# shadimsaleh/motion_detection

Measured on AMD Instinct MI355X. Metric: Mpixels/s (flow+warp+diff) at 1080p & 4K; % HBM roofline, 1/2/4/8 GPU, higher is better.
Workload: dtype u8

## Files before the change

motion_detection_amd/csrc/mdx_api.cpp:

```cpp
#include "mdx_ctx.h"

#include <cstdlib>
#include <map>
#include <mutex>

using namespace mdx;

static thread_local std::string g_create_err;

extern "C" void mdx_default_params(mdx_params* p)
{
    p->win = 40;
    p->max_level = 5;
    p->max_iters = 10;
    p->eps = 0.03;
    p->min_eig = 0.001f;
    p->thresh = 190;
    p->pixel_step = 10;
    p->min_vector_size = 1.0;
    p->fit_mode = MDX_FIT_FIRST4;
    p->subspace_precision = MDX_SUBSPACE_F64;
    p->call_pipelining = 0;
    p->ransac_iters = 128;
    p->ransac_thresh = 3.0;
    p->ransac_seed = 20141105u;
}

extern "C" int mdx_grid_count(int w, int h, int ps)
{
    if (w <= 0 || h <= 0 || ps <= 0) return 0;
    return ((w + ps - 1) / ps) * ((h + ps - 1) / ps);
}

static const char* check_params(const mdx_params* p)
{
    if (p->win != kWin) return "only win == 40 (the reference constant) is supported";
    if (p->max_level < 0 || p->max_level >= kMaxLevels) return "max_level out of range [0, 7]";
    if (p->pixel_step <= 0) return "pixel_step must be > 0 (reference leaves it unset: UB)";
    if (p->fit_mode != MDX_FIT_FIRST4 && p->fit_mode != MDX_FIT_EXTERNAL && p->fit_mode != MDX_FIT_RANSAC) return "bad fit_mode";
    if (p->ransac_iters < 1 || p->ransac_iters > kRansacMaxIters) return "ransac_iters must be in [1, 1024]";
    if (!(p->ransac_thresh >= 0.0) || !(p->ransac_thresh < 1e6)) return "ransac_thresh must be in [0, 1e6)";
    if (p->subspace_precision != MDX_SUBSPACE_F64 && p->subspace_precision != MDX_SUBSPACE_F32) return "bad subspace_precision";
    if (p->call_pipelining != 0 && p->call_pipelining != 1) return "call_pipelining must be 0 or 1";
    return nullptr;
}

static std::mutex g_host_mu;
static std::map<uintptr_t, size_t> g_host_blocks;
bool mdx::host_block_holds(const void* p, size_t bytes)
{
    const uintptr_t a = reinterpret_cast<uintptr_t>(p);
    std::lock_guard<std::mutex> lk(g_host_mu);
    auto it = g_host_blocks.upper_bound(a);
    if (it == g_host_blocks.begin()) return false;
    --it;
    return a >= it->first && bytes <= it->second && a - it->first <= it->second - bytes;
}

extern "C" const char* mdx_create_error(void) { return g_create_err.c_str(); }
extern "C" int mdx_abi_version(void) { return MDX_ABI_VERSION; }
extern "C" size_t mdx_params_size(void) { return sizeof(mdx_params); }

static LkTuning read_tuning()
{
    LkTuning t;
    auto num = [](const char* name, int dflt) {
        const char* e = std::getenv(name);
        return e ? std::atoi(e) : dflt;
    };
    t.lk_impl = num("MDX_LK_IMPL", 2) == 1 ? 1 : 2;
    t.lk_g = num("MDX_LK_G", 0);
    t.lk_sub = num("MDX_LK_SUB", 0);
    t.lk_astrip = std::max(0, std::min(num("MDX_LK_ASTRIP", 0), 64));
    t.lk_debug = num("MDX_LK_DEBUG", 0) != 0;
    t.traj_chain = num("MDX_TRAJ_CHAIN", 1) != 0;
    const int ppw = num("MDX_TRAJ_PPW", 4);
    t.traj_ppw = ppw == 1 ? 1 : ppw == 2 ? 2 : 4;
    t.lk_aux = num("MDX_LK_AUX", 1) != 0;
    t.lk_flow = num("MDX_LK_FLOW", 1) != 0;
    t.ol_reg = num("MDX_OL_REG", 1) != 0;
    t.lk_cap = std::min(std::max(num("MDX_LK_CAP", 75), 10), 100);
    t.lk_fma = num("MDX_LK_FMA", 1) != 0;
    t.spin_max = num("MDX_LK_SPIN_MAX", kLkSpinDefault);
    return t;
}

static bool new_stream(mdx_ctx* c, hipStream_t* s)
{
    if (hipStreamCreateWithFlags(s, hipStreamNonBlocking) != hipSuccess) {
        *s = nullptr;
        return false;
    }
    c->streams.push_back(*s);
    return true;
}

static bool new_events(mdx_ctx* c, hipEvent_t* e, int n, unsigned flags = hipEventDisableTiming)
{
    for (int i = 0; i < n; i++) {
        if (hipEventCreateWithFlags(&e[i], flags) != hipSuccess) return false;
        c->events.push_back(e[i]);
    }
    return true;
}

extern "C" mdx_ctx* mdx_create(int device, int max_w, int max_h, int max_batch, const mdx_params* p)
{
    g_create_err.clear();
    mdx_params prm;
    if (p) prm = *p;
    else mdx_default_params(&prm);
    if (const char* why = check_params(&prm)) { g_create_err = why; return nullptr; }
    if (max_w <= 0 || max_h <= 0 || max_batch <= 0) { g_create_err = "max_w/max_h/max_batch must be > 0"; return nullptr; }
    int ndev = 0;
    if (hipGetDeviceCount(&ndev) != hipSuccess || ndev == 0) { g_create_err = "no HIP device visible"; return nullptr; }
    if (device < 0 || device >= ndev) { g_create_err = "device index out of range"; return nullptr; }
    if (hipSetDevice(device) != hipSuccess) { g_create_err = "hipSetDevice failed"; return nullptr; }
    mdx_ctx* c = new mdx_ctx();
    c->device = device;
    c->prm = prm;
    c->max_w = max_w;
    c->max_h = max_h;
    c->max_batch = max_batch;
    static_cast<LkTuning&>(*c) = read_tuning();
    auto fail = [&](const std::string& msg) -> mdx_ctx* {
// ... 310 lines not shown
```

motion_detection_amd/csrc/mdx_ctx.h:

```cpp
#pragma once

#include "../../include/mdx.h"
#include "mdx_internal.h"

#include <algorithm>
#include <array>
#include <cstdarg>
#include <cstdio>
#include <initializer_list>
#include <string>
#include <utility>
#include <vector>

struct DevBuf {
    void* p = nullptr;
    size_t cap = 0;
    DevBuf() = default;
    DevBuf(DevBuf&& o) noexcept : p(std::exchange(o.p, nullptr)), cap(std::exchange(o.cap, 0)) {}
    DevBuf& operator=(DevBuf&& o) noexcept
    {
        std::swap(p, o.p), std::swap(cap, o.cap);
        return *this;
    }
    ~DevBuf() { reset(); }
    void reset()
    {
        if (p) (void)hipFree(p);
        p = nullptr, cap = 0;
    }
    bool alloc(size_t bytes)
    {
        reset();
        if (hipMalloc(&p, bytes) != hipSuccess) p = nullptr;
        cap = p ? bytes : 0;
        return p != nullptr;
    }
    template <typename T> T* as() const { return static_cast<T*>(p); }
};

struct LkTuning {
    int lk_impl = 2;
    int lk_g = 0;
    int lk_sub = 0;
    int lk_astrip = 0;
    bool lk_debug = false;
    bool traj_chain = true;
    int traj_ppw = 4;
    bool lk_aux = true;
    bool lk_flow = true;
    int lk_cap = 75;
    bool lk_fma = true;
    int spin_max = mdx::kLkSpinDefault;
    bool ol_reg = true;
};

struct mdx_ctx : LkTuning {
    int device = 0;
    std::vector<hipStream_t> streams;
    std::vector<hipEvent_t> events;
    std::vector<void*> pinned;
    hipStream_t stream = nullptr;
    hipStream_t aux = nullptr;
    hipEvent_t lkev[mdx::kMaxLevels + 2] = {};
    hipStream_t iter2 = nullptr;
    hipEvent_t flowev[2] = {};
    hipEvent_t front_ev = nullptr;
    hipEvent_t pyr_free[2] = {};
    hipEvent_t lvl_done[mdx::kMaxLevels] = {};
    hipEvent_t redo_ev[mdx::kMaxLevels] = {};
    mdx::LkLaunch lk;
    int pyr_half = 0;
    hipEvent_t input_ev = nullptr;
    uint8_t* last_pyr1 = nullptr;
    uint8_t* last_pyr2 = nullptr;
    uint8_t* band_pyr1 = nullptr;
    uint8_t* band_pyr2 = nullptr;
    int band_half = 0;
    const uint8_t* band_img1 = nullptr;
    int band_built[2] = {0, 0};
    int band_stride = 0, band_fmt = 0;
    DevBuf errw;
    int* err_host = nullptr;
    int* tcnt_host = nullptr;
    long long lk_fallback[3] = {0, 0, 0};
    mdx_params prm{};
    int max_w = 0, max_h = 0, max_batch = 0;
    DevBuf pyr1, pyr2, der, fits;
    DevBuf in1, in2, np, st, vec, mask, H, Hext, num;
    DevBuf bnp, bst;
    DevBuf cls, Abuf, ctab;
    DevBuf dbg;
    DevBuf lkcnt;
    DevBuf csum;
    DevBuf tin, tcur, tnp, tst, ttraj, tnum, tflag;
    DevBuf straj, sdata, sq, scnt, scols, sres, sout, sbest;
    DevBuf clpts, clbest, clroot;
// ... 145 lines not shown
```

motion_detection_amd/csrc/mdx_dev.h:

```cpp
#pragma once

#include "mdx_internal.h"

namespace mdx {

__device__ __forceinline__ int r101(int p, int len)
{
    if ((unsigned)p < (unsigned)len) return p;
    if (len == 1) return 0;
    do {
        if (p < 0) p = -p;
        else p = 2 * len - 2 - p;
    } while ((unsigned)p >= (unsigned)len);
    return p;
}

struct __attribute__((aligned(4))) u4a4k { uint32_t x, y, z, w; };
struct __attribute__((aligned(4))) u3a4k { uint32_t x, y, z; };
struct __attribute__((aligned(4))) u2a4k { uint32_t x, y; };
template <typename T>
__device__ __forceinline__ T gload(uintptr_t a)
{
#if defined(__HIP_DEVICE_COMPILE__)
    return *reinterpret_cast<const __attribute__((address_space(1))) T*>(a);
#else
    return *reinterpret_cast<const T*>(a);
#endif
}

template <int T>
__device__ __forceinline__ int block_scan_exclusive(int v, int* wsum, int& total)
{
    const int lane = threadIdx.x & 63, w = threadIdx.x >> 6;
    int inc = v;
#pragma unroll
    for (int d = 1; d < 64; d <<= 1) {
        const int o = __shfl_up(inc, d, 64);
        if (lane >= d) inc += o;
    }
    if (lane == 63) wsum[w] = inc;
    __syncthreads();
    int off = 0, tot = 0;
#pragma unroll
    for (int i = 0; i < T / 64; i++) {
        const int s = wsum[i];
        if (i < w) off += s;
        tot += s;
    }
    __syncthreads();
    total = tot;
    return off + inc - v;
}

__device__ __forceinline__ int u8_at(const uint32_t (&w)[3], int b) { return (int)((w[b >> 2] >> (8 * (b & 3))) & 255u); }

__device__ __forceinline__ uint32_t scharr_word(const uint32_t (&ra)[3], const uint32_t (&rb)[3], const uint32_t (&rc)[3],
                                                int bc)
{
    const int bm = bc - 1, bp = bc + 1;
    const int t0m = (u8_at(ra, bm) + u8_at(rc, bm)) * 3 + u8_at(rb, bm) * 10;
    const int t0p = (u8_at(ra, bp) + u8_at(rc, bp)) * 3 + u8_at(rb, bp) * 10;
    const int t1m = u8_at(rc, bm) - u8_at(ra, bm), t1c = u8_at(rc, bc) - u8_at(ra, bc), t1p = u8_at(rc, bp) - u8_at(ra, bp);
    const int ix = t0p - t0m;
    const int iy = (t1m + t1p) * 3 + t1c * 10;
    return (uint32_t)(uint16_t)(int16_t)ix | ((uint32_t)(uint16_t)(int16_t)iy << 16);
}

__device__ __forceinline__ int gray_of(const uint8_t* s, int fmt)
{
    if (fmt == 1) return (s[0] * 1868 + s[1] * 9617 + s[2] * 4899 + 8192) >> 14;
    return (s[2] * 1868 + s[1] * 9617 + s[0] * 4899 + 8192) >> 14;
}

__device__ __forceinline__ void gray_chunk(const uint8_t* s, int px0, int w, int fmt, uint32_t (&o)[4])
{
    if (px0 >= 0 && px0 + 16 <= w && fmt == 0 && (((uintptr_t)(s + px0)) & 3) == 0) {
        const u4a4k v = *reinterpret_cast<const u4a4k*>(s + px0);
        o[0] = v.x; o[1] = v.y; o[2] = v.z; o[3] = v.w;
    } else if (px0 >= 0 && px0 + 16 <= w && fmt != 0 && (((uintptr_t)(s + 3 * px0)) & 3) == 0) {
        uint32_t b[12];
        const u4a4k* q = reinterpret_cast<const u4a4k*>(s + 3 * px0);
#pragma unroll
        for (int t = 0; t < 3; t++) { const u4a4k v = q[t]; b[4 * t] = v.x; b[4 * t + 1] = v.y; b[4 * t + 2] = v.z; b[4 * t + 3] = v.w; }
        const uint8_t* bb = reinterpret_cast<const uint8_t*>(b);
#pragma unroll
        for (int t = 0; t < 4; t++) {
            uint32_t d = 0;
#pragma unroll
            for (int i = 0; i < 4; i++) d |= (uint32_t)gray_of(bb + 3 * (4 * t + i), fmt) << (8 * i);
            o[t] = d;
        }
    } else {
        for (int t = 0; t < 4; t++) {
            uint32_t d = 0;
            for (int i = 0; i < 4; i++) {
                const int px = px0 + 4 * t + i;
                if (px < -kPad || px >= w + kPad) continue;
                const int sx = r101(px, w);
                d |= (uint32_t)(fmt == 0 ? s[sx] : gray_of(s + 3 * sx, fmt)) << (8 * i);
            }
            o[t] = d;
        }
    }
}

}
```

motion_detection_amd/csrc/mdx_internal.h:

```cpp
#pragma once

#include <hip/hip_runtime.h>
#include <math.h>
#include <stdint.h>

#include <algorithm>

#include "mdx.h"
#include "mdx_plan.h"

namespace mdx {

static_assert(sizeof(float4) == kFloat4Bytes, "lk_scratch sizes the A sums by it");
constexpr int kLkDbgStampOff = kMaxLevels * 64 + 64;
constexpr int kLkDbgWaves = 16384;

inline uint8_t* level0_core(uint8_t* slab, const Geometry& g) { return slab + g.lv[0].img_off + g.lv[0].core(); }

struct PairFit {
    double H[9];
    double Hinv[9];
    int num_vectors;
    int fit_status;
    int src_y0, src_y1;
};

struct LkClassArgs {
    Geometry g;
    ClassPlan plan;
    const int16_t* rlist;
    int level;
};

struct LkArgs {
    const uint8_t* pyr1;
    const uint8_t* pyr2;
    const uint32_t* der;
    Geometry g;
    int maxl;
    int npts, ny, pixel_step;
    int nyg;
    int max_iters;
    float min_eig;
    double eps2;
    float* next_pts;
    float* carry;
    long long carry_lstride;
    uint8_t* status;
    ClassPlan plan;
    const int16_t* cmap;
    const int16_t* rlist;
    const int16_t* ord;
    const float* prev_pts;
    int max_sub;
    int* done;
    int done_stride;
    int dep_groups;
    int* err;
    int* lflags;
    int redo;
    int spin_max;
    int flow_cap;
    float4* dbg;
    int dbg_pt;
    int fma;
    uint32_t* body_cnt;
};

constexpr int kLkSpinDefault = 1 << 19;
#ifndef MDX_LK_REDO_WAVES
#define MDX_LK_REDO_WAVES 512
#endif
constexpr int kLkRedoWaves = MDX_LK_REDO_WAVES;

hipError_t launch_gray_pad(hipStream_t s, int batch, const uint8_t* in1, const uint8_t* in2, int w, int h,
                           int stride, long long frame_stride, int fmt, uint8_t* pyr1, uint8_t* pyr2,
                           const Geometry& g, int fsel = 0);
hipError_t launch_front(hipStream_t s, int batch, const uint8_t* in1, const uint8_t* in2, int w, int h, int stride,
                        long long frame_stride, int fmt, uint8_t* pyr1, uint8_t* pyr2, const Geometry& g,
                        int fsel = 0, const RowSpan* rows = nullptr);
hipError_t launch_pyr_levels(hipStream_t s, int batch, uint8_t* pyr1, uint8_t* pyr2, const Geometry& g, int fsel = 0,
                             const RowSpan* rows = nullptr);
hipError_t launch_scharr_levels(hipStream_t s, int batch, const uint8_t* pyr1, uint32_t* der, const Geometry& g);
hipError_t launch_scharr(hipStream_t s, int batch, const uint8_t* pyr1, uint32_t* der, const Geometry& g, int level,
                         int prow0 = 0, int prow1 = -1);
hipError_t launch_lk(hipStream_t s, int batch, const LkArgs& a);

constexpr int kMaxTrajImgs = 16;
struct TrajChain {
    const uint8_t* pyr[kMaxTrajImgs];
    const uint32_t* der[kMaxTrajImgs];
    int nimg, w, h;
    float* cur;
    float* traj;
    int* tlen;
    int* flag;
    double* vectors;
    float* start_pts;
    int* num;
    double mvs;
    float* htraj;
    int* htlen;
    float* hstart;
    double* hvec;
};
hipError_t launch_lk_chain(hipStream_t s, const LkArgs& a, const TrajChain& t, int ppw);
size_t subspace_basis_bytes(int n, int d, int precision);
// ... 165 lines not shown
```

motion_detection_amd/csrc/mdx_lk.hip:

```cpp
#include "mdx_dev.h"

#include <float.h>

#include <algorithm>
#include <atomic>
#include <cstdlib>
#include <type_traits>

namespace mdx {

typedef short s2 __attribute__((ext_vector_type(2)));
typedef float f2 __attribute__((ext_vector_type(2)));
typedef unsigned int v4u __attribute__((ext_vector_type(4)));
typedef unsigned int v3u __attribute__((ext_vector_type(3)));
struct LkRunRsrc {
    unsigned long long base;
    uint32_t bytes;

    __device__ __forceinline__ LkRunRsrc(const void* p, uint32_t n)
    {
        const unsigned long long b = (unsigned long long)(uintptr_t)p;
        const uint32_t lo = __builtin_amdgcn_readfirstlane((uint32_t)b);
        const uint32_t hi = __builtin_amdgcn_readfirstlane((uint32_t)(b >> 32)) & 0xffffu;
        base = ((unsigned long long)hi << 32) | lo;
        bytes = __builtin_amdgcn_readfirstlane(n);
    }
    __device__ __forceinline__ void advance(uint32_t step)
    {
        base += step;
        bytes -= step;
        asm("" : "+s"(base), "+s"(bytes));
    }
    __device__ __forceinline__ __amdgpu_buffer_rsrc_t rsrc() const
    {
        const v4u w = {(uint32_t)base, (uint32_t)(base >> 32), bytes, 0x00020000u};
        __amdgpu_buffer_rsrc_t r;
        static_assert(sizeof(r) == sizeof(w), "descriptor words");
        __builtin_memcpy(&r, &w, sizeof(r));
        return r;
    }
};

__device__ __forceinline__ int class_of(const int16_t* cmap, int level, int axis, int res)
{
    return cmap[(level * 2 + axis) * kTabStride + res];
}
__device__ __forceinline__ int residue_of(const int16_t* rlist, int level, int axis, int cls)
{
    return rlist[(level * 2 + axis) * kTabStride + cls];
}

__device__ __forceinline__ void lk_weights(float fa, float fb, int& w00, int& w01, int& w10, int& w11)
{
    w00 = __float2int_rn((1.f - fa) * (1.f - fb) * 16384.f);
    w01 = __float2int_rn(fa * (1.f - fb) * 16384.f);
    w10 = __float2int_rn((1.f - fa) * fb * 16384.f);
    w11 = 16384 - w00 - w01 - w10;
}

template <int Q>
__device__ __forceinline__ void lk_interp(uint32_t lo0, uint32_t hi0, uint32_t lo1, uint32_t hi1, uint32_t d00,
                                          uint32_t d01, uint32_t d10, uint32_t d11, s2 W0, s2 W1, int& ival, int& ixv,
                                          int& iyv)
{
    static_assert(Q >= 0 && Q < 7, "tap byte");
    constexpr unsigned sel = 0x0c000c00u | (unsigned)Q | ((unsigned)(Q + 1) << 16);
    const s2 t0 = __builtin_bit_cast(s2, __builtin_amdgcn_perm(hi0, lo0, sel));
    const s2 t1 = __builtin_bit_cast(s2, __builtin_amdgcn_perm(hi1, lo1, sel));
    ival = __builtin_amdgcn_sdot2(t0, W0, __builtin_amdgcn_sdot2(t1, W1, 256, false), false) >> 9;
    const s2 x0 = __builtin_bit_cast(s2, __builtin_amdgcn_perm(d01, d00, 0x05040100u));
    const s2 x1 = __builtin_bit_cast(s2, __builtin_amdgcn_perm(d11, d10, 0x05040100u));
    const s2 y0 = __builtin_bit_cast(s2, __builtin_amdgcn_perm(d01, d00, 0x07060302u));
    const s2 y1 = __builtin_bit_cast(s2, __builtin_amdgcn_perm(d11, d10, 0x07060302u));
    ixv = __builtin_amdgcn_sdot2(x0, W0, __builtin_amdgcn_sdot2(x1, W1, 8192, false), false) >> 14;
    iyv = __builtin_amdgcn_sdot2(y0, W0, __builtin_amdgcn_sdot2(y1, W1, 8192, false), false) >> 14;
}

template <int J>
__device__ __forceinline__ float quad_bcast(float v)
{
    constexpr int ctrl = J | (J << 2) | (J << 4) | (J << 6);
    return __int_as_float(__builtin_amdgcn_mov_dpp(__float_as_int(v), ctrl, 0xf, 0xf, false));
}
template <int J>
__device__ __forceinline__ uint32_t quad_bcast_u(uint32_t v)
{
    constexpr int ctrl = J | (J << 2) | (J << 4) | (J << 6);
    return (uint32_t)__builtin_amdgcn_mov_dpp((int)v, ctrl, 0xf, 0xf, false);
}

__device__ __forceinline__ void wave_lds_fence()
{
    __builtin_amdgcn_fence(__ATOMIC_RELEASE, "wavefront");
    __builtin_amdgcn_wave_barrier();
    __builtin_amdgcn_fence(__ATOMIC_ACQUIRE, "wavefront");
}

constexpr int kLkIterWavesPerEU = 4;
typedef __attribute__((address_space(3))) void* lds_ptr;
typedef __attribute__((address_space(3))) uint32_t lds_u32;
typedef unsigned int v2u __attribute__((ext_vector_type(2)));
typedef __attribute__((address_space(3))) volatile const v2u lds_u2v;
typedef __attribute__((address_space(3))) volatile const v4u lds_u4v;
__device__ __forceinline__ void lk_vmcnt0()
{
    __builtin_amdgcn_sched_barrier(0);
    __builtin_amdgcn_s_waitcnt(0x0F70);
    __builtin_amdgcn_sched_barrier(0);
}
template <int N>
__device__ __forceinline__ void lk_vmcnt()
{
    static_assert(N >= 0 && N < 16, "vmcnt field");
    __builtin_amdgcn_sched_barrier(0);
    __builtin_amdgcn_s_waitcnt(0x0F70 | N);
    __builtin_amdgcn_sched_barrier(0);
}

template <int B, int E, typename F>
__device__ __forceinline__ void static_for(F&& f)
{
    if constexpr (B < E) {
        f(std::integral_constant<int, B>{});
        static_for<B + 1, E>(f);
    }
}

__device__ __forceinline__ int xcd_remap(int b, int total)
{
    const int xcd = b & 7, q = total >> 3, r = total & 7;
    return (xcd < r ? xcd * (q + 1) : r * (q + 1) + (xcd - r) * q) + (b >> 3);
}

__device__ __forceinline__ void cls_store(uint4* o, const uint32_t (&dv)[4], const int (&cv)[4])
{
    typedef unsigned v4nt __attribute__((ext_vector_type(4)));
    const uint4 a = make_uint4(dv[0], (uint32_t)cv[0], dv[1], (uint32_t)cv[1]);
    const uint4 b = make_uint4(dv[2], (uint32_t)cv[2], dv[3], (uint32_t)cv[3]);
    __builtin_nontemporal_store(__builtin_bit_cast(v4nt, a), reinterpret_cast<v4nt*>(o));
    __builtin_nontemporal_store(__builtin_bit_cast(v4nt, b), reinterpret_cast<v4nt*>(o) + 1);
}

__global__ __launch_bounds__(256) void k_lk_class(const uint8_t* __restrict__ pyr1, const uint32_t* __restrict__ der,
                                                  uint8_t* __restrict__ cls_out, LkClassArgs a)
{
    const int level = a.level;
    const ClassLevel& C = a.plan.lv[level];
    const int nclass = C.nrx * C.nry;
    const int pair = blockIdx.z / nclass, cls = blockIdx.z % nclass;
    const int j = blockIdx.x * blockDim.x + threadIdx.x;
    const int v = C.vlo + blockIdx.y;
    if (4 * j >= a.g.lv[level].w + 2 * kPad || v >= C.UH) return;
    const Level L = a.g.lv[level];
    const float scale = (float)(1. / (1 << level));
    const int rx = residue_of(a.rlist, level, 0, cls % C.nrx), ry = residue_of(a.rlist, level, 1, cls / C.nrx);
    const float ppx = (float)rx * scale - 19.5f, ppy = (float)ry * scale - 19.5f;
    const float fa = ppx - floorf(ppx), fb = ppy - floorf(ppy);
    int w00, w01, w10, w11;
    lk_weights(fa, fb, w00, w01, w10, w11);
    const uint8_t* I = pyr1 + (long long)pair * a.g.img_bytes + L.img_off + L.core();
    const uint32_t* D = der + (long long)pair * a.g.der_words + L.der_off + L.core();
    const int y = v - kPad;
    const int p = L.pitch;
    uint8_t* base = cls_out + (long long)pair * a.plan.bytes_per_pair + C.off + (long long)cls * C.class_bytes;
    uint32_t dv[4] = {0, 0, 0, 0};
    int cv[4];
    const int x0 = 4 * j - kPad;
    if (y < L.h + kPad - 1 && x0 < L.w + kPad - 1) {
        const uint8_t* ip = I + (long long)y * p + x0;
        const uint32_t* dp = D + (long long)y * p + x0;
        uint32_t ib[2][2], dw[2][5];
#pragma unroll
        for (int r = 0; r < 2; r++) {
            const u2a4k bi = *reinterpret_cast<const u2a4k*>(ip + (long long)r * p);
            ib[r][0] = bi.x; ib[r][1] = bi.y;
            const uint4 d4 = *reinterpret_cast<const uint4*>(dp + (long long)r * p);
            dw[r][0] = d4.x; dw[r][1] = d4.y; dw[r][2] = d4.z; dw[r][3] = d4.w;
            dw[r][4] = dp[(long long)r * p + 4];
        }
        const s2 W0 = {(short)w00, (short)w01}, W1 = {(short)w10, (short)w11};
        static_for<0, 4>([&](auto qc) {
            constexpr int q = decltype(qc)::value;
            if (x0 + q >= L.w + kPad - 1) { cv[q] = 256; return; }
            int ival, ixv, iyv;
            lk_interp<q>(ib[0][0], ib[0][1], ib[1][0], ib[1][1], dw[0][q], dw[0][q + 1], dw[1][q], dw[1][q + 1], W0, W1,
                         ival, ixv, iyv);
            dv[q] = ((uint32_t)ixv & 0xffffu) | ((uint32_t)iyv << 16);
            cv[q] = 256 - 512 * ival;
        });
    } else {
#pragma unroll
        for (int q = 0; q < 4; q++) cv[q] = 256;
    }
    uint4* o = reinterpret_cast<uint4*>(base) + ((long long)v * C.PW + 4 * j) / 2;
    cls_store(o, dv, cv);
}

__global__ __launch_bounds__(256) void k_lk_class_fused(const uint8_t* __restrict__ pyr1, uint8_t* __restrict__ cls_out,
                                                        LkClassArgs a)
{
    const int level = a.level;
    const ClassLevel& C = a.plan.lv[level];
    const int nclass = C.nrx * C.nry;
    const int pair = blockIdx.z;
    const int j = blockIdx.x * blockDim.x + threadIdx.x;
    const int v = C.vlo + blockIdx.y;
    if (4 * j >= a.g.lv[level].w + 2 * kPad || v >= C.UH) return;
    const Level L = a.g.lv[level];
    const float scale = (float)(1. / (1 << level));
    const uint8_t* I = pyr1 + (long long)pair * a.g.img_bytes + L.img_off + L.core();
    const int y = v - kPad;
    const int p = L.pitch;
    const int x0 = 4 * j - kPad;
    const bool inside = y < L.h + kPad - 1 && x0 < L.w + kPad - 1;
    uint32_t rw[4][3];
#pragma unroll
    for (int r = 0; r < 4; r++) {
        const int yy = y - 1 + r;
        const int ys = (yy < -kPad || yy >= L.h + kPad) ? y : yy;
        const u3a4k t = *reinterpret_cast<const u3a4k*>(I + (long long)ys * p + x0 - 4);
        rw[r][0] = t.x; rw[r][1] = t.y; rw[r][2] = t.z;
    }
    uint32_t dw[2][5];
#pragma unroll
    for (int r = 0; r < 2; r++) {
        const int yy = y + r;
#pragma unroll
        for (int c = 0; c < 5; c++) {
            const int x = x0 + c;
            const bool in = yy >= 0 && yy < L.h && x >= 0 && x < L.w;
            dw[r][c] = in ? scharr_word(rw[r], rw[r + 1], rw[r + 2], 4 + c) : 0u;
        }
    }
    for (int cls = 0; cls < nclass; cls++) {
        const int rx = residue_of(a.rlist, level, 0, cls % C.nrx), ry = residue_of(a.rlist, level, 1, cls / C.nrx);
        const float ppx = (float)rx * scale - 19.5f, ppy = (float)ry * scale - 19.5f;
        const float fa = ppx - floorf(ppx), fb = ppy - floorf(ppy);
        int w00, w01, w10, w11;
        lk_weights(fa, fb, w00, w01, w10, w11);
        uint32_t dv[4] = {0, 0, 0, 0};
        int cv[4] = {256, 256, 256, 256};
        if (inside) {
            const s2 W0 = {(short)w00, (short)w01}, W1 = {(short)w10, (short)w11};
            static_for<0, 4>([&](auto qc) {
                constexpr int q = decltype(qc)::value;
                if (x0 + q >= L.w + kPad - 1) return;
                int ival, ixv, iyv;
                lk_interp<q>(rw[1][1], rw[1][2], rw[2][1], rw[2][2], dw[0][q], dw[0][q + 1], dw[1][q], dw[1][q + 1], W0,
                             W1, ival, ixv, iyv);
                dv[q] = ((uint32_t)ixv & 0xffffu) | ((uint32_t)iyv << 16);
                cv[q] = 256 - 512 * ival;
            });
        }
        uint8_t* base = cls_out + (long long)pair * a.plan.bytes_per_pair + C.off + (long long)cls * C.class_bytes;
        uint4* o = reinterpret_cast<uint4*>(base) + ((long long)v * C.PW + 4 * j) / 2;
        cls_store(o, dv, cv);
    }
}

template <int G, int UW>
struct LkShape {
    static constexpr int UWIDTH = UW;
    static constexpr int LPS = 4 * G;
    static constexpr int S = 64 / LPS;
    static constexpr int NP = (UW + 2 * LPS - 1) / (2 * LPS);
    static constexpr int BYTES = S * UW * 8;
    static constexpr int ND = (BYTES + 1023) / 1024;
    static_assert(UW % 2 == 0 && UW >= kWin, "union width");
};

struct GroupGeom {
    int gx, gy;
    bool valid;
    int ipx, ipy;
    int off;
    int v0;
    uint32_t ubase;
};

template <int G, int UW>
__device__ __forceinline__ GroupGeom group_geom(const LkArgs& a, const ClassLevel& C, int level, int g, int sl)
{
    GroupGeom r;
    const int16_t* xo = a.ord + C.ord_off;
    const int16_t* yo = xo + C.nxp;
    const bool has = g >= 0;
    const int gg = has ? g : 0;
    const int cg = gg / a.nyg, row = gg - cg * a.nyg;
    const int e0 = cg * G;
    const int gxv = has ? xo[e0 + (sl >> 2)] : -1;
    r.valid = gxv >= 0;
    r.gx = r.valid ? gxv : 0;
    r.gy = yo[row];
    r.ipx = lk_win_origin(r.gx, a.pixel_step, level);
    r.ipy = lk_win_origin(r.gy, a.pixel_step, level);
    const int gx0 = has ? xo[e0] : 0;
    const int ipx0 = lk_win_origin(gx0, a.pixel_step, level);
    const int m = (1 << level) - 1;
    const int cx = class_of(a.cmap, level, 0, (gx0 * a.pixel_step) & m);
    const int cy = class_of(a.cmap, level, 1, (r.gy * a.pixel_step) & m);
    const int ub = min(max(ipx0 + kPad, 0), C.PW - UW);
    r.off = min(max(r.ipx + kPad - ub, 0), UW - kWin);
    r.v0 = lk_win_row0(r.ipy, C.UH);
    r.ubase = (uint32_t)(C.off + (long long)(cy * C.nrx + cx) * C.class_bytes) + 8u * (uint32_t)ub;
    return r;
}

template <typename Sh>
__device__ __forceinline__ void lk_piece_offsets(uint32_t mine, int lane, uint32_t (&uoff)[Sh::ND])
// ... 647 lines not shown
    const dim3 grid((ngroups + S - 1) / S, batch);
    hipLaunchKernelGGL((k_lk_A<G, UW>), grid, dim3(64), 0, s, a, cls, Ab, cert, qctr, l, ngroups);
}

template <int G, int UW>
static void launch_A_rows(hipStream_t s, int batch, const LkArgs& a, const uint8_t* cls, float4* Ab, uint8_t* cert,
                          int* qctr, int l)
{
    constexpr int S = LkShape<G, UW>::S;
    const ClassLevel& C = a.plan.lv[l];
    const int ncg = C.nxp / G;
    const dim3 grid(((ncg + S - 1) / S) * C.nstrip, batch);
    if (C.asp >= 10)
        hipLaunchKernelGGL((k_lk_A_rows<G, UW, 4>), grid, dim3(64), 0, s, a, cls, Ab, cert, qctr, l, ncg);
    else
        hipLaunchKernelGGL((k_lk_A_rows<G, UW, 8>), grid, dim3(64), 0, s, a, cls, Ab, cert, qctr, l, ncg);
}

template <int G, int UW>
static void launch_iter(hipStream_t s, int batch, const LkArgs& a, const uint8_t* cls, const float4* Ab,
                        const uint8_t* cert, int* qctr, int l)
{
    constexpr int S = LkShape<G, UW>::S;
    const int ngroups = lk_groups(a.plan, l, a.nyg);
    const int need = (int)std::min<long long>(((long long)batch * ngroups + S - 1) / S, 1 << 30);
    const bool df = a.done || a.redo || a.lflags || a.dep_groups;
    int res = df ? lk_iter_resident<G, UW, true>() : lk_iter_resident<G, UW, false>();
    if (a.done) res = res * std::min(std::max(a.flow_cap, 10), 100) / 100;
    int W = std::max(8, std::min((need + 7) / 8, res / 8) * 8);
    if (a.redo) W = std::max(8, std::min(W, kLkRedoWaves));
    if (df)
        hipLaunchKernelGGL((k_lk_iter<G, UW, true>), dim3(W), dim3(64), 0, s, a, cls, Ab, cert, qctr, l, ngroups, batch);
    else
        hipLaunchKernelGGL((k_lk_iter<G, UW, false>), dim3(W), dim3(64), 0, s, a, cls, Ab, cert, qctr, l, ngroups, batch);
}

static bool launch_level(bool iter, hipStream_t st, int batch, const LkArgs& a, const uint8_t* cls, float4* Ab,
                         uint8_t* cert, int* qctr, int l)
{
    const ClassLevel& C = a.plan.lv[l];
    switch (C.G * 1000 + C.UW) {
#define LK_CASE(g, uw)                                                   \
    case g * 1000 + uw:                                                  \
        if (iter) launch_iter<g, uw>(st, batch, a, cls, Ab, cert, qctr, l);    \
        else if (C.asp) launch_A_rows<g, uw>(st, batch, a, cls, Ab, cert, qctr, l); \
        else launch_A<g, uw>(st, batch, a, cls, Ab, cert, qctr, l);            \
        return true;
        LK_SHAPES
#undef LK_CASE
    default: return false;
    }
}

static hipError_t lk_enqueue_planes(const LkLaunch& L, hipStream_t sa, int batch, int p, int nb, const LkArgs& a,
                                    const LkArgs& b, uint8_t* bcls, int* bq)
{
    if (L.aux) {
        hipEvent_t ready = L.prev_ready;
        if (!ready || p) {
            if (hipError_t e = hipEventRecord(L.ev[kMaxLevels], L.s)) return e;
            ready = L.ev[kMaxLevels];
        }
        if (hipError_t e = hipStreamWaitEvent(sa, ready, 0)) return e;
    }
    for (int l = a.maxl; l >= 0; l--) {
        const ClassLevel& C = a.plan.lv[l];
        if (L.aux && L.lvl_done) {
            if (hipError_t e = hipStreamWaitEvent(sa, L.lvl_done[l], 0)) return e;
        }
        LkClassArgs ca;
        ca.g = a.g;
        ca.plan = a.plan;
        ca.rlist = a.rlist;
        ca.level = l;
        if (C.nrx * C.nry <= 4) {
            const dim3 grid(((a.g.lv[l].w + 2 * kPad) / 4 + 63) / 64, C.vhi - C.vlo, nb);
            hipLaunchKernelGGL(k_lk_class_fused, grid, dim3(64), 0, sa, b.pyr1, bcls, ca);
        } else {
            const dim3 grid(((a.g.lv[l].w + 2 * kPad) / 4 + 63) / 64, C.vhi - C.vlo, nb * C.nrx * C.nry);
            if (hipError_t e = launch_scharr(sa, nb, b.pyr1, const_cast<uint32_t*>(b.der), a.g, l, C.vlo, C.vhi + 1))
                return e;
            hipLaunchKernelGGL(k_lk_class, grid, dim3(64), 0, sa, b.pyr1, b.der, bcls, ca);
        }
        float4* bA = L.Ab + ((long long)l * batch + p) * a.npts;
        uint8_t* bC = L.cert + ((long long)l * batch + p) * a.npts;
        if (!launch_level(false, sa, nb, b, bcls, bA, bC, bq, l)) return hipErrorInvalidValue;
        if (L.aux) {
            if (hipError_t e = hipEventRecord(L.ev[l], sa)) return e;
        }
    }
    return hipSuccess;
}

static hipError_t lk_enqueue_iters(const LkLaunch& L, int batch, int p, int nb, const LkArgs& a, const LkArgs& b,
                                   uint8_t* bcls, int* bq)
{
    const bool flow_ok = L.aux && L.s2 && L.flow_ev && L.done && L.redo_ev && a.err && b.carry &&
                         (reinterpret_cast<uintptr_t>(b.carry) & 127) == 0 && (a.carry_lstride % 32) == 0;
    const bool flow = flow_ok && nb % 8 == 0 && nb >= 16 && a.npts % 16 == 0 &&
                      (reinterpret_cast<uintptr_t>(b.next_pts) & 127) == 0;
    int* lflags = flow ? L.done + (long long)kMaxLevels * nb * kCtrPad : nullptr;
    if (flow) {
        if (hipError_t e = hipMemsetAsync(L.done, 0, sizeof(int) * ((long long)kMaxLevels * nb + kLkFlagInts) * kCtrPad, L.s))
            return e;
        if (hipError_t e = hipEventRecord(L.flow_ev[0], L.s)) return e;
        if (hipError_t e = hipStreamWaitEvent(L.s2, L.flow_ev[0], 0)) return e;
    }
    for (int l = a.maxl; l >= 0; l--) {
        hipStream_t st = flow && ((a.maxl - l) & 1) ? L.s2 : L.s;
        if (L.aux) {
            if (hipError_t e = hipStreamWaitEvent(st, L.ev[l], 0)) return e;
        }
        LkArgs bl = b;
        bl.done = flow ? L.done : nullptr;
        bl.done_stride = nb;
        bl.dep_groups = 0;
        bl.lflags = lflags;
        bl.redo = 0;
        if (flow && l < a.maxl) {
            const int ngc = lk_groups(a.plan, l + 1, a.nyg), ng = lk_groups(a.plan, l, a.nyg);
            bl.dep_groups = ngc;
            hipLaunchKernelGGL(k_lk_gate, dim3(1), dim3(64), 0, st, bq + (l + 1) * 8 * kCtrPad, (long long)nb * ngc,
                               L.done + (l + 1) * nb * kCtrPad, bl.dep_groups, ng, (long long)nb * ng, a.err,
                               a.spin_max, lflags + (kLkFlagGiveup + l) * kCtrPad);
        }
        float4* bA = L.Ab + ((long long)l * batch + p) * a.npts;
        uint8_t* bC = L.cert + ((long long)l * batch + p) * a.npts;
        if (!launch_level(true, st, nb, bl, bcls, bA, bC, bq, l)) return hipErrorInvalidValue;
        if (flow) {
            if (l < a.maxl) {
                if (hipError_t e = hipStreamWaitEvent(st, L.redo_ev[l + 1], 0)) return e;
                LkArgs br = bl;
                br.done = nullptr;
                br.dep_groups = 0;
                br.redo = 1;
// ... 44 lines not shown
```

motion_detection_amd/csrc/mdx_pair.cpp:

```cpp
#include "mdx_ctx.h"

#include <cmath>
#include <cstdlib>
#include <new>

using namespace mdx;

static int ensure_class_plan(mdx_ctx* c, const Geometry& g, int w, int h, int ps, int batch, int gy0, int gy1)
{
    int rc;
    const std::array<int, 6> key = {w, h, ps, g.nlev, gy0, gy1};
    if (c->plan_key != key) {
        BuiltPlan B;
        try {
            B = build_class_plan(g, w, h, ps, gy0, gy1, PlanTuning{c->lk_g, c->lk_astrip, c->max_batch});
        } catch (const std::bad_alloc&) {
            return set_err(c, MDX_ENOMEM, "class plan: out of host memory");
        }
        if ((rc = ensure(c, c->ctab, B.tab.size() * sizeof(int16_t))) != MDX_OK) return rc;
        HIP_OR_RETURN(c, hipStreamSynchronize(c->stream));
        HIP_OR_RETURN(c, hipMemcpy(c->ctab.p, B.tab.data(), B.tab.size() * sizeof(int16_t), hipMemcpyHostToDevice));
        c->plan = B.plan;
        c->plan_key = key;
    }
    if (c->plan.nch == 0) return MDX_OK;
    return ensure(c, c->cls, (size_t)c->plan.bytes_per_pair * batch + 64);
}

static int wait_input(mdx_ctx* c, hipStream_t st)
{
    if (!c->input_ev) return MDX_OK;
    hipEvent_t e = c->input_ev;
    c->input_ev = nullptr;
    HIP_OR_RETURN(c, hipStreamWaitEvent(st, e, 0));
    return MDX_OK;
}

int mdx::run_lk(mdx_ctx* c, const Geometry& g, LkArgs& a, int batch, int w, int h, int gy0, int gy1, bool have_scharr,
                hipEvent_t prev_ready)
{
    int rc;
    hipStream_t s = c->stream;
    bool v2 = c->lk_impl == 2 && a.prev_pts == nullptr;
    if (v2) {
        if ((rc = ensure_class_plan(c, g, w, h, c->prm.pixel_step, batch, gy0, gy1)) != MDX_OK) return rc;
        v2 = c->plan.nch != 0;
    }
    if (!v2) {
        if (gy0 != 0 || gy1 != a.ny)
            return set_err(c, MDX_EINVAL, "row bands need the class-plane LK (pixel_step too large)");
        if (!have_scharr) HIP_OR_RETURN(c, launch_scharr_levels(s, batch, a.pyr1, const_cast<uint32_t*>(a.der), g));
        HIP_OR_RETURN(c, launch_lk(s, batch, a));
        return MDX_OK;
    }
    a.plan = c->plan;
    a.max_sub = c->lk_sub;
    a.err = c->errw.as<int>();
    a.spin_max = c->spin_max;
    a.flow_cap = c->lk_cap;
    a.fma = c->lk_fma ? 1 : 0;
    a.cmap = c->ctab.as<int16_t>();
    a.rlist = c->ctab.as<int16_t>() + kTabRlist;
    a.ord = c->ctab.as<int16_t>() + kTabOrd;
    const int npts = a.npts;
    if (c->lk_debug) {
        if ((rc = ensure(c, c->dbg, ((size_t)npts * g.nlev * batch + kLkDbgStampOff + kMaxLevels * kLkDbgWaves) * 16)) !=
            MDX_OK)
            return rc;
        a.dbg = c->dbg.as<float4>();
        const char* e = std::getenv("MDX_LK_DEBUG_PT");
        a.dbg_pt = e ? std::atoi(e) : -1;
        if ((rc = ensure(c, c->lkcnt, kMaxLevels * 2 * sizeof(uint32_t))) != MDX_OK) return rc;
        HIP_OR_RETURN(c, hipMemsetAsync(c->lkcnt.p, 0, kMaxLevels * 2 * sizeof(uint32_t), s));
        a.body_cnt = c->lkcnt.as<uint32_t>();
    }
    const LkScratch sc = lk_scratch(g.nlev, batch, npts);
    if ((rc = ensure(c, c->Abuf, sc.bytes)) != MDX_OK) return rc;
    const std::array<size_t, 4> lay = {reinterpret_cast<size_t>(c->Abuf.p), (size_t)g.nlev, (size_t)batch, (size_t)npts};
    if (c->lk_scratch_key != lay) {
        HIP_OR_RETURN(c, hipStreamSynchronize(c->stream));
        c->lk_scratch_key = lay;
    }
    uint8_t* base = c->Abuf.as<uint8_t>();
    a.carry = reinterpret_cast<float*>(base + sc.carry);
    a.carry_lstride = (long long)(sc.carry_level / sizeof(float));
    LkLaunch L = c->lk;
    L.cls = c->cls.as<uint8_t>();
    L.Ab = c->Abuf.as<float4>();
    L.cert = base + sc.cert;
    L.qctr = reinterpret_cast<int*>(base + sc.qctr);
    L.done = reinterpret_cast<int*>(base + sc.done);
    L.lvl_done = c->prm.call_pipelining ? c->lvl_done : nullptr;
    L.prev_ready = prev_ready;
    HIP_OR_RETURN(c, launch_lk_v2(L, batch, a));
    return MDX_OK;
}

static int run_warp_diff(mdx_ctx* c, int batch, const WarpArgs& a)
{
    const size_t wsb = warp_scratch_bytes(batch, a.w, (a.row1 < 0 ? a.h : a.row1) - a.row0);
    if (const int rc = ensure(c, c->wscr, wsb); rc != MDX_OK) return rc;
    HIP_OR_RETURN(c, launch_warp_diff(c->stream, batch, a, c->wscr.p, wsb, &c->last_warp));
    return MDX_OK;
}
static GrayPlane pyr_gray(uint8_t* slab, const Geometry& g)
{
    return {level0_core(slab, g), g.img_bytes, g.lv[0].pitch};
}

// ... 284 lines not shown
```

Before: 9191.

## Walk multiple rows per thread in class-plane LK kernels with shared weight tables

The class-plane kernels now let each thread walk R consecutive rows, reusing the previous row's interpolation pairs and the rolling Scharr input rows instead of reloading two or four rows for every output row. The per-class bilinear weights are computed once per block, in shared memory for the generic kernel and in registers for the fused one, and one block loops over many classes instead of launching one block per class. A wave-count heuristic chooses the row count and class split, with an environment override. The risk is lower parallelism and more register use at small levels, plus more complex boundary handling through perm selector masks.

```diff
diff --git a/motion_detection_amd/csrc/mdx_api.cpp b/motion_detection_amd/csrc/mdx_api.cpp
--- a/motion_detection_amd/csrc/mdx_api.cpp
+++ b/motion_detection_amd/csrc/mdx_api.cpp
@@ -71,6 +71,7 @@
     t.lk_impl = num("MDX_LK_IMPL", 2) == 1 ? 1 : 2;
     t.lk_g = num("MDX_LK_G", 0);
     t.lk_sub = num("MDX_LK_SUB", 0);
+    t.lk_class_rows = std::max(0, num("MDX_LK_CLASS_ROWS", 0));
     t.lk_astrip = std::max(0, std::min(num("MDX_LK_ASTRIP", 0), 64));
     t.lk_debug = num("MDX_LK_DEBUG", 0) != 0;
     t.traj_chain = num("MDX_TRAJ_CHAIN", 1) != 0;
diff --git a/motion_detection_amd/csrc/mdx_ctx.h b/motion_detection_amd/csrc/mdx_ctx.h
--- a/motion_detection_amd/csrc/mdx_ctx.h
+++ b/motion_detection_amd/csrc/mdx_ctx.h
@@ -42,6 +42,7 @@
     int lk_impl = 2;
     int lk_g = 0;
     int lk_sub = 0;
+    int lk_class_rows = 0;
     int lk_astrip = 0;
     bool lk_debug = false;
     bool traj_chain = true;
diff --git a/motion_detection_amd/csrc/mdx_dev.h b/motion_detection_amd/csrc/mdx_dev.h
--- a/motion_detection_amd/csrc/mdx_dev.h
+++ b/motion_detection_amd/csrc/mdx_dev.h
@@ -54,16 +54,30 @@
 
 __device__ __forceinline__ int u8_at(const uint32_t (&w)[3], int b) { return (int)((w[b >> 2] >> (8 * (b & 3))) & 255u); }
 
-__device__ __forceinline__ uint32_t scharr_word(const uint32_t (&ra)[3], const uint32_t (&rb)[3], const uint32_t (&rc)[3],
-                                                int bc)
+__device__ __forceinline__ void scharr_ixiy(const uint32_t (&ra)[3], const uint32_t (&rb)[3], const uint32_t (&rc)[3],
+                                            int bc, int& ix, int& iy)
 {
     const int bm = bc - 1, bp = bc + 1;
     const int t0m = (u8_at(ra, bm) + u8_at(rc, bm)) * 3 + u8_at(rb, bm) * 10;
     const int t0p = (u8_at(ra, bp) + u8_at(rc, bp)) * 3 + u8_at(rb, bp) * 10;
     const int t1m = u8_at(rc, bm) - u8_at(ra, bm), t1c = u8_at(rc, bc) - u8_at(ra, bc), t1p = u8_at(rc, bp) - u8_at(ra, bp);
-    const int ix = t0p - t0m;
-    const int iy = (t1m + t1p) * 3 + t1c * 10;
+    ix = t0p - t0m;
+    iy = (t1m + t1p) * 3 + t1c * 10;
+}
+
+__device__ __forceinline__ uint32_t scharr_word(const uint32_t (&ra)[3], const uint32_t (&rb)[3], const uint32_t (&rc)[3],
+                                                int bc)
+{
+    int ix, iy;
+    scharr_ixiy(ra, rb, rc, bc, ix, iy);
     return (uint32_t)(uint16_t)(int16_t)ix | ((uint32_t)(uint16_t)(int16_t)iy << 16);
+}
+
+__device__ __forceinline__ void scharr_row5(const uint32_t (&ra)[3], const uint32_t (&rb)[3], const uint32_t (&rc)[3],
+                                            int (&ix)[5], int (&iy)[5])
+{
+#pragma unroll
+    for (int c = 0; c < 5; c++) scharr_ixiy(ra, rb, rc, 4 + c, ix[c], iy[c]);
 }
 
 __device__ __forceinline__ int gray_of(const uint8_t* s, int fmt)
diff --git a/motion_detection_amd/csrc/mdx_internal.h b/motion_detection_amd/csrc/mdx_internal.h
--- a/motion_detection_amd/csrc/mdx_internal.h
+++ b/motion_detection_amd/csrc/mdx_internal.h
@@ -53,6 +53,7 @@
     const int16_t* ord;
     const float* prev_pts;
     int max_sub;
+    int class_rows;
     int* done;
     int done_stride;
     int dep_groups;
diff --git a/motion_detection_amd/csrc/mdx_lk.hip b/motion_detection_amd/csrc/mdx_lk.hip
--- a/motion_detection_amd/csrc/mdx_lk.hip
+++ b/motion_detection_amd/csrc/mdx_lk.hip
@@ -58,22 +58,33 @@
     w11 = 16384 - w00 - w01 - w10;
 }
 
-template <int Q>
-__device__ __forceinline__ void lk_interp(uint32_t lo0, uint32_t hi0, uint32_t lo1, uint32_t hi1, uint32_t d00,
-                                          uint32_t d01, uint32_t d10, uint32_t d11, s2 W0, s2 W1, int& ival, int& ixv,
-                                          int& iyv)
-{
-    static_assert(Q >= 0 && Q < 7, "tap byte");
-    constexpr unsigned sel = 0x0c000c00u | (unsigned)Q | ((unsigned)(Q + 1) << 16);
-    const s2 t0 = __builtin_bit_cast(s2, __builtin_amdgcn_perm(hi0, lo0, sel));
-    const s2 t1 = __builtin_bit_cast(s2, __builtin_amdgcn_perm(hi1, lo1, sel));
-    ival = __builtin_amdgcn_sdot2(t0, W0, __builtin_amdgcn_sdot2(t1, W1, 256, false), false) >> 9;
-    const s2 x0 = __builtin_bit_cast(s2, __builtin_amdgcn_perm(d01, d00, 0x05040100u));
-    const s2 x1 = __builtin_bit_cast(s2, __builtin_amdgcn_perm(d11, d10, 0x05040100u));
-    const s2 y0 = __builtin_bit_cast(s2, __builtin_amdgcn_perm(d01, d00, 0x07060302u));
-    const s2 y1 = __builtin_bit_cast(s2, __builtin_amdgcn_perm(d11, d10, 0x07060302u));
-    ixv = __builtin_amdgcn_sdot2(x0, W0, __builtin_amdgcn_sdot2(x1, W1, 8192, false), false) >> 14;
-    iyv = __builtin_amdgcn_sdot2(y0, W0, __builtin_amdgcn_sdot2(y1, W1, 8192, false), false) >> 14;
+struct LkRowPairs {
+    s2 t[4], x[4], y[4];
+};
+__device__ __forceinline__ uint32_t lk_tap_sel(int q) { return 0x0c000c00u | (unsigned)q | ((unsigned)(q + 1) << 16); }
+constexpr uint32_t kLkSelLo = 0x05040100u, kLkSelHi = 0x07060302u, kLkSelZero = 0x0c0c0c0cu;
+__device__ __forceinline__ s2 lk_perm(uint32_t hi, uint32_t lo, uint32_t sel)
+{
+    return __builtin_bit_cast(s2, __builtin_amdgcn_perm(hi, lo, sel));
+}
+__device__ __forceinline__ void lk_interp(const LkRowPairs& a, const LkRowPairs& b, int q, s2 W0, s2 W1, uint32_t& d, int& c)
+{
+    const int ival = __builtin_amdgcn_sdot2(a.t[q], W0, __builtin_amdgcn_sdot2(b.t[q], W1, 256, false), false) >> 9;
+    const int ixv = __builtin_amdgcn_sdot2(a.x[q], W0, __builtin_amdgcn_sdot2(b.x[q], W1, 8192, false), false) >> 14;
+    const int iyv = __builtin_amdgcn_sdot2(a.y[q], W0, __builtin_amdgcn_sdot2(b.y[q], W1, 8192, false), false) >> 14;
+    d = ((uint32_t)ixv & 0xffffu) | ((uint32_t)iyv << 16);
+    c = 256 - 512 * ival;
+}
+__device__ __forceinline__ void lk_class_weights(const int16_t* rlist, int level, int nrx, int cls, s2& W0, s2& W1)
+{
+    const float scale = (float)(1. / (1 << level));
+    const int rx = residue_of(rlist, level, 0, cls % nrx), ry = residue_of(rlist, level, 1, cls / nrx);
+    const float ppx = (float)rx * scale - 19.5f, ppy = (float)ry * scale - 19.5f;
+    const float fa = ppx - floorf(ppx), fb = ppy - floorf(ppy);
+    int w00, w01, w10, w11;
+    lk_weights(fa, fb, w00, w01, w10, w11);
+    W0 = s2{(short)w00, (short)w01};
+    W1 = s2{(short)w10, (short)w11};
 }
 
 template <int J>
@@ -141,120 +152,156 @@
     __builtin_nontemporal_store(__builtin_bit_cast(v4nt, b), reinterpret_cast<v4nt*>(o) + 1);
 }
 
-__global__ __launch_bounds__(256) void k_lk_class(const uint8_t* __restrict__ pyr1, const uint32_t* __restrict__ der,
-                                                  uint8_t* __restrict__ cls_out, LkClassArgs a)
-{
+__device__ __forceinline__ void lk_class_row(const LkRowPairs& a, const LkRowPairs& b, s2 W0, s2 W1, uint8_t* o)
+{
+    uint32_t dv[4];
+    int cv[4];
+#pragma unroll
+    for (int q = 0; q < 4; q++) lk_interp(a, b, q, W0, W1, dv[q], cv[q]);
+    cls_store(reinterpret_cast<uint4*>(o), dv, cv);
+}
+
+__global__ __launch_bounds__(64) void k_lk_class(const uint8_t* __restrict__ pyr1, const uint32_t* __restrict__ der,
+                                                 uint8_t* __restrict__ cls_out, LkClassArgs a, int R, int cpp, int nsplit)
+{
+    __shared__ uint32_t wtab[2 * 64];
     const int level = a.level;
     const ClassLevel& C = a.plan.lv[level];
     const int nclass = C.nrx * C.nry;
-    const int pair = blockIdx.z / nclass, cls = blockIdx.z % nclass;
+    const int pair = blockIdx.z / nsplit, c0 = (blockIdx.z % nsplit) * cpp;
+    const int nc = min(cpp, nclass - c0);
+    if ((int)threadIdx.x < nc) {
+        s2 W0, W1;
+        lk_class_weights(a.rlist, level, C.nrx, c0 + threadIdx.x, W0, W1);
+        wtab[2 * threadIdx.x] = __builtin_bit_cast(uint32_t, W0);
+        wtab[2 * threadIdx.x + 1] = __builtin_bit_cast(uint32_t, W1);
+    }
+    __syncthreads();
     const int j = blockIdx.x * blockDim.x + threadIdx.x;
-    const int v = C.vlo + blockIdx.y;
-    if (4 * j >= a.g.lv[level].w + 2 * kPad || v >= C.UH) return;
+    const int v0 = C.vlo + blockIdx.y * R;
+    const int nrows = min(R, min(C.vhi, C.UH) - v0);
     const Level L = a.g.lv[level];
-    const float scale = (float)(1. / (1 << level));
-    const int rx = residue_of(a.rlist, level, 0, cls % C.nrx), ry = residue_of(a.rlist, level, 1, cls / C.nrx);
-    const float ppx = (float)rx * scale - 19.5f, ppy = (float)ry * scale - 19.5f;
-    const float fa = ppx - floorf(ppx), fb = ppy - floorf(ppy);
-    int w00, w01, w10, w11;
-    lk_weights(fa, fb, w00, w01, w10, w11);
-    const uint8_t* I = pyr1 + (long long)pair * a.g.img_bytes + L.img_off + L.core();
-    const uint32_t* D = der + (long long)pair * a.g.der_words + L.der_off + L.core();
-    const int y = v - kPad;
+    if (4 * j >= L.w + 2 * kPad || nrows <= 0) return;
     const int p = L.pitch;
-    uint8_t* base = cls_out + (long long)pair * a.plan.bytes_per_pair + C.off + (long long)cls * C.class_bytes;
-    uint32_t dv[4] = {0, 0, 0, 0};
-    int cv[4];
     const int x0 = 4 * j - kPad;
-    if (y < L.h + kPad - 1 && x0 < L.w + kPad - 1) {
-        const uint8_t* ip = I + (long long)y * p + x0;
-        const uint32_t* dp = D + (long long)y * p + x0;
-        uint32_t ib[2][2], dw[2][5];
-#pragma unroll
-        for (int r = 0; r < 2; r++) {
-            const u2a4k bi = *reinterpret_cast<const u2a4k*>(ip + (long long)r * p);
-            ib[r][0] = bi.x; ib[r][1] = bi.y;
-            const uint4 d4 = *reinterpret_cast<const uint4*>(dp + (long long)r * p);
-            dw[r][0] = d4.x; dw[r][1] = d4.y; dw[r][2] = d4.z; dw[r][3] = d4.w;
-            dw[r][4] = dp[(long long)r * p + 4];
-        }
-        const s2 W0 = {(short)w00, (short)w01}, W1 = {(short)w10, (short)w11};
-        static_for<0, 4>([&](auto qc) {
-            constexpr int q = decltype(qc)::value;
-            if (x0 + q >= L.w + kPad - 1) { cv[q] = 256; return; }
-            int ival, ixv, iyv;
-            lk_interp<q>(ib[0][0], ib[0][1], ib[1][0], ib[1][1], dw[0][q], dw[0][q + 1], dw[1][q], dw[1][q + 1], W0, W1,
-                         ival, ixv, iyv);
-            dv[q] = ((uint32_t)ixv & 0xffffu) | ((uint32_t)iyv << 16);
-            cv[q] = 256 - 512 * ival;
-        });
-    } else {
-#pragma unroll
-        for (int q = 0; q < 4; q++) cv[q] = 256;
-    }
-    uint4* o = reinterpret_cast<uint4*>(base) + ((long long)v * C.PW + 4 * j) / 2;
-    cls_store(o, dv, cv);
-}
-
-__global__ __launch_bounds__(256) void k_lk_class_fused(const uint8_t* __restrict__ pyr1, uint8_t* __restrict__ cls_out,
-                                                        LkClassArgs a)
+    const bool act = x0 < L.w + kPad - 1;
+    uint32_t tsel[4], xsel[4], ysel[4];
+#pragma unroll
+    for (int q = 0; q < 4; q++) {
+        const bool ok = x0 + q < L.w + kPad - 1;
+        tsel[q] = ok ? lk_tap_sel(q) : kLkSelZero;
+        xsel[q] = ok ? kLkSelLo : kLkSelZero;
+        ysel[q] = ok ? kLkSelHi : kLkSelZero;
+    }
+    const long long row0 = (long long)(v0 - kPad) * p + x0;
+    const uint8_t* ip = pyr1 + (long long)pair * a.g.img_bytes + L.img_off + L.core() + row0;
+    const uint32_t* dp = der + (long long)pair * a.g.der_words + L.der_off + L.core() + row0;
+    auto row_pairs = [&](LkRowPairs& P) {
+        uint32_t i0 = 0, i1 = 0, dw[5] = {0, 0, 0, 0, 0};
+        if (act) {
+            const u2a4k bi = *reinterpret_cast<const u2a4k*>(ip);
+            const uint4 d4 = *reinterpret_cast<const uint4*>(dp);
+            i0 = bi.x; i1 = bi.y;
+            dw[0] = d4.x; dw[1] = d4.y; dw[2] = d4.z; dw[3] = d4.w;
+            dw[4] = dp[4];
+        }
+        ip += p;
+        dp += p;
+#pragma unroll
+        for (int q = 0; q < 4; q++) {
+            P.t[q] = lk_perm(i1, i0, tsel[q]);
+            P.x[q] = lk_perm(dw[q + 1], dw[q], xsel[q]);
+            P.y[q] = lk_perm(dw[q + 1], dw[q], ysel[q]);
+        }
+    };
+    uint8_t* orow = cls_out + (long long)pair * a.plan.bytes_per_pair + C.off + (long long)c0 * C.class_bytes +
+                    ((long long)v0 * C.PW + 4 * j) * 8;
+    LkRowPairs A, B;
+    row_pairs(A);
+    for (int s = 0; s < nrows; s++) {
+        row_pairs(B);
+        uint8_t* o = orow;
+        for (int c = 0; c < nc; c++) {
+            const s2 W0 = __builtin_bit_cast(s2, wtab[2 * c]), W1 = __builtin_bit_cast(s2, wtab[2 * c + 1]);
+            lk_class_row(A, B, W0, W1, o);
+            o += C.class_bytes;
+        }
+        orow += (long long)C.PW * 8;
+        A = B;
+    }
+}
+
+template <int R, int NC>
+__global__ __launch_bounds__(64) void k_lk_class_fused(const uint8_t* __restrict__ pyr1, uint8_t* __restrict__ cls_out,
+                                                       LkClassArgs a)
 {
     const int level = a.level;
     const ClassLevel& C = a.plan.lv[level];
     const int nclass = C.nrx * C.nry;
     const int pair = blockIdx.z;
     const int j = blockIdx.x * blockDim.x + threadIdx.x;
-    const int v = C.vlo + blockIdx.y;
-    if (4 * j >= a.g.lv[level].w + 2 * kPad || v >= C.UH) return;
+    const int v0 = C.vlo + blockIdx.y * R;
+    const int nrows = min(R, min(C.vhi, C.UH) - v0);
     const Level L = a.g.lv[level];
-    const float scale = (float)(1. / (1 << level));
-    const uint8_t* I = pyr1 + (long long)pair * a.g.img_bytes + L.img_off + L.core();
-    const int y = v - kPad;
+    if (4 * j >= L.w + 2 * kPad || nrows <= 0) return;
+    s2 W0[NC], W1[NC];
+#pragma unroll
+    for (int c = 0; c < NC; c++) {
+        W0[c] = W1[c] = s2{0, 0};
+        if (c < nclass) lk_class_weights(a.rlist, level, C.nrx, c, W0[c], W1[c]);
+    }
     const int p = L.pitch;
     const int x0 = 4 * j - kPad;
-    const bool inside = y < L.h + kPad - 1 && x0 < L.w + kPad - 1;
-    uint32_t rw[4][3];
-#pragma unroll
-    for (int r = 0; r < 4; r++) {
-        const int yy = y - 1 + r;
-        const int ys = (yy < -kPad || yy >= L.h + kPad) ? y : yy;
-        const u3a4k t = *reinterpret_cast<const u3a4k*>(I + (long long)ys * p + x0 - 4);
-        rw[r][0] = t.x; rw[r][1] = t.y; rw[r][2] = t.z;
-    }
-    uint32_t dw[2][5];
-#pragma unroll
-    for (int r = 0; r < 2; r++) {
-        const int yy = y + r;
-#pragma unroll
-        for (int c = 0; c < 5; c++) {
-            const int x = x0 + c;
-            const bool in = yy >= 0 && yy < L.h && x >= 0 && x < L.w;
-            dw[r][c] = in ? scharr_word(rw[r], rw[r + 1], rw[r + 2], 4 + c) : 0u;
-        }
-    }
-    for (int cls = 0; cls < nclass; cls++) {
-        const int rx = residue_of(a.rlist, level, 0, cls % C.nrx), ry = residue_of(a.rlist, level, 1, cls / C.nrx);
-        const float ppx = (float)rx * scale - 19.5f, ppy = (float)ry * scale - 19.5f;
-        const float fa = ppx - floorf(ppx), fb = ppy - floorf(ppy);
-        int w00, w01, w10, w11;
-        lk_weights(fa, fb, w00, w01, w10, w11);
-        uint32_t dv[4] = {0, 0, 0, 0};
-        int cv[4] = {256, 256, 256, 256};
-        if (inside) {
-            const s2 W0 = {(short)w00, (short)w01}, W1 = {(short)w10, (short)w11};
-            static_for<0, 4>([&](auto qc) {
-                constexpr int q = decltype(qc)::value;
-                if (x0 + q >= L.w + kPad - 1) return;
-                int ival, ixv, iyv;
-                lk_interp<q>(rw[1][1], rw[1][2], rw[2][1], rw[2][2], dw[0][q], dw[0][q + 1], dw[1][q], dw[1][q + 1], W0,
-                             W1, ival, ixv, iyv);
-                dv[q] = ((uint32_t)ixv & 0xffffu) | ((uint32_t)iyv << 16);
-                cv[q] = 256 - 512 * ival;
-            });
-        }
-        uint8_t* base = cls_out + (long long)pair * a.plan.bytes_per_pair + C.off + (long long)cls * C.class_bytes;
-        uint4* o = reinterpret_cast<uint4*>(base) + ((long long)v * C.PW + 4 * j) / 2;
-        cls_store(o, dv, cv);
+    uint32_t tsel[4], dsel[4];
+#pragma unroll
+    for (int q = 0; q < 4; q++) {
+        const int x = x0 + q;
+        tsel[q] = x < L.w + kPad - 1 ? lk_tap_sel(q) : kLkSelZero;
+        dsel[q] = (x >= 0 && x < L.w ? 0x0100u : 0x0c0cu) | (x + 1 >= 0 && x + 1 < L.w ? 0x05040000u : 0x0c0c0000u);
+    }
+    const uint8_t* I = pyr1 + (long long)pair * a.g.img_bytes + L.img_off + L.core() + x0 - 4;
+    auto load_row = [&](int yy, uint32_t (&r)[3]) {
+        const int ys = min(max(yy, -kPad), L.h + kPad - 1);
+        const u3a4k t = *reinterpret_cast<const u3a4k*>(I + (long long)ys * p);
+        r[0] = t.x; r[1] = t.y; r[2] = t.z;
+    };
+    auto row_pairs = [&](int yy, const uint32_t (&ra)[3], const uint32_t (&rb)[3], const uint32_t (&rc)[3], LkRowPairs& P) {
+#pragma unroll
+        for (int q = 0; q < 4; q++) {
+            P.t[q] = lk_perm(rb[2], rb[1], tsel[q]);
+            P.x[q] = P.y[q] = s2{0, 0};
+        }
+        if (yy >= 0 && yy < L.h) {
+            int ix[5], iy[5];
+            scharr_row5(ra, rb, rc, ix, iy);
+#pragma unroll
+            for (int q = 0; q < 4; q++) {
+                P.x[q] = lk_perm((uint32_t)ix[q + 1], (uint32_t)ix[q], dsel[q]);
+                P.y[q] = lk_perm((uint32_t)iy[q + 1], (uint32_t)iy[q], dsel[q]);
+            }
+        }
+    };
+    const int y0 = v0 - kPad;
+    uint32_t ra[3], rb[3], rc[3], rn[3];
+    load_row(y0 - 1, ra);
+    load_row(y0, rb);
+    load_row(y0 + 1, rc);
+    load_row(y0 + 2, rn);
+    LkRowPairs A, B;
+    row_pairs(y0, ra, rb, rc, A);
+    uint8_t* orow = cls_out + (long long)pair * a.plan.bytes_per_pair + C.off + ((long long)v0 * C.PW + 4 * j) * 8;
+#pragma unroll
+    for (int s = 0; s < R; s++) {
+        if (s >= nrows) break;
+#pragma unroll
+        for (int i = 0; i < 3; i++) { ra[i] = rb[i]; rb[i] = rc[i]; rc[i] = rn[i]; }
+        if (s + 1 < R) load_row(y0 + s + 3, rn);
+        row_pairs(y0 + s + 1, ra, rb, rc, B);
+#pragma unroll
+        for (int c = 0; c < NC; c++)
+            if (c < nclass) lk_class_row(A, B, W0[c], W1[c], orow + (long long)c * C.class_bytes);
+        orow += (long long)C.PW * 8;
+        A = B;
     }
 }
 
@@ -1008,6 +1055,11 @@
     }
 }
 
+constexpr int kLkFusedRows = 8;
+constexpr int kLkClassMinWaves = 4096;
+constexpr int kLkClassSplitWaves = 16384;
+static long long lk_class_waves(int gx, int nrows, int R, int nz) { return (long long)gx * ((nrows + R - 1) / R) * nz; }
+
 static hipError_t lk_enqueue_planes(const LkLaunch& L, hipStream_t sa, int batch, int p, int nb, const LkArgs& a,
                                     const LkArgs& b, uint8_t* bcls, int* bq)
 {
@@ -1029,14 +1081,28 @@
         ca.plan = a.plan;
         ca.rlist = a.rlist;
         ca.level = l;
-        if (C.nrx * C.nry <= 4) {
-            const dim3 grid(((a.g.lv[l].w + 2 * kPad) / 4 + 63) / 64, C.vhi - C.vlo, nb);
-            hipLaunchKernelGGL(k_lk_class_fused, grid, dim3(64), 0, sa, b.pyr1, bcls, ca);
+        const int nclass = C.nrx * C.nry, gx = ((a.g.lv[l].w + 2 * kPad) / 4 + 63) / 64, nrows = C.vhi - C.vlo;
+        if (nclass <= 4) {
+            const bool walk = a.class_rows ? a.class_rows > 1 : lk_class_waves(gx, nrows, kLkFusedRows, nb) >= kLkClassMinWaves;
+            const int R = walk ? kLkFusedRows : 1;
+            const dim3 grid(gx, (nrows + R - 1) / R, nb);
+            if (R > 1 && nclass == 1) hipLaunchKernelGGL((k_lk_class_fused<kLkFusedRows, 1>), grid, dim3(64), 0, sa, b.pyr1, bcls, ca);
+            else if (R > 1) hipLaunchKernelGGL((k_lk_class_fused<kLkFusedRows, 4>), grid, dim3(64), 0, sa, b.pyr1, bcls, ca);
+            else if (nclass == 1) hipLaunchKernelGGL((k_lk_class_fused<1, 1>), grid, dim3(64), 0, sa, b.pyr1, bcls, ca);
+            else hipLaunchKernelGGL((k_lk_class_fused<1, 4>), grid, dim3(64), 0, sa, b.pyr1, bcls, ca);
         } else {
-            const dim3 grid(((a.g.lv[l].w + 2 * kPad) / 4 + 63) / 64, C.vhi - C.vlo, nb * C.nrx * C.nry);
+            int R = 4, nsplit = (nclass + 63) / 64;
+            const long long floor_waves = a.class_rows > 1 ? 0 : kLkClassSplitWaves;
+            if (a.class_rows == 1) R = 1;
+            while (R > 1 && lk_class_waves(gx, nrows, R, nb * nsplit) < floor_waves) R /= 2;
+            while (nsplit < nclass && lk_class_waves(gx, nrows, R, nb * nsplit) < floor_waves) nsplit *= 2;
+            nsplit = std::min(nsplit, nclass);
+            const int cpp = (nclass + nsplit - 1) / nsplit;
+            nsplit = (nclass + cpp - 1) / cpp;
+            const dim3 grid(gx, (nrows + R - 1) / R, nb * nsplit);
             if (hipError_t e = launch_scharr(sa, nb, b.pyr1, const_cast<uint32_t*>(b.der), a.g, l, C.vlo, C.vhi + 1))
                 return e;
-            hipLaunchKernelGGL(k_lk_class, grid, dim3(64), 0, sa, b.pyr1, b.der, bcls, ca);
+            hipLaunchKernelGGL(k_lk_class, grid, dim3(64), 0, sa, b.pyr1, b.der, bcls, ca, R, cpp, nsplit);
         }
         float4* bA = L.Ab + ((long long)l * batch + p) * a.npts;
         uint8_t* bC = L.cert + ((long long)l * batch + p) * a.npts;
diff --git a/motion_detection_amd/csrc/mdx_pair.cpp b/motion_detection_amd/csrc/mdx_pair.cpp
--- a/motion_detection_amd/csrc/mdx_pair.cpp
+++ b/motion_detection_amd/csrc/mdx_pair.cpp
@@ -55,6 +55,7 @@
     }
     a.plan = c->plan;
     a.max_sub = c->lk_sub;
+    a.class_rows = c->lk_class_rows;
     a.err = c->errw.as<int>();
     a.spin_max = c->spin_max;
     a.flow_cap = c->lk_cap;
```

Result: no change. 9189, median of 2 (-0.0%).
